# imedslab/OAProgressionMMF

Hardware: AMD Instinct MI355X
Metric: knees/sec full XR+MRI+clin fusion train step (higher is better)
Workload: dtype f32; 1 GPU; syn3: XR1MR3C1CnnTrf train step (fwd+FocalLoss+bwd+Adam), per-GPU batch 8, global batch 8, BASELINE config 4 on BASELINE's synthetic tensors: XR 1x310x310 + 3 x MRI 1x160x384x384 (slice-major) + 9 clinical; random-init weights; parallelism=dp1, activation_recompute=012,012,01

## Files before the change

### oaprogressionmmf_amd/csrc/koaf_conv.hip

```cpp
#include "koaf_common.h"

namespace {

inline int64_t rup32(int64_t v) { return (v + 31) / 32 * 32; }

inline void set_fimg(KoafGemm* g, const KoafWImg* w, int R, int64_t K) {
    g->fmt = 1;
    g->A.fscale = KOAF_ACT_SCALE;
    g->B.amax = w->amax;
    if (!w->f) return;
    g->B.kind = 2; g->B.gather = 0;
    g->B.planes = w->f; g->B.ld = rup32(K); g->B.plane_stride = (int64_t)R * g->B.ld;
}

inline void set_aplanes(KoafOperand* a, const uint16_t* planes, int64_t plane_elems) {
    a->kind = 2; a->planes = planes; a->plane_stride = plane_elems; a->zeros = planes + 2 * plane_elems;
    a->ptr = nullptr; a->ptr2 = nullptr; a->tf = 0; a->sc = a->sh = a->sc2 = nullptr;
}

inline void set_gather(KoafOperand* o, int gather, int H, int W, int C, int CS, int PH, int PW, int KH, int KW, int stride, int pad_h,
                       int pad_w) {
    o->gather = gather;
    o->H = H; o->W = W; o->C = C; o->CS = CS;
    o->PH = PH; o->PW = PW;
    o->KH = KH; o->KW = KW; o->stride = stride; o->pad = pad_h; o->pad_w = pad_w;
}

inline bool is_pointwise(int KH, int KW, int stride, int pad) { return KH == 1 && KW == 1 && stride == 1 && pad == 0; }

struct WgradPlan { int bm, bn, splitk; };
inline WgradPlan wgrad_plan(int M, int N, int64_t K, int ctap, int batch) {
    WgradPlan p;
    p.bn = (N >= 128 && (ctap % 4) == 0) ? 128 : 64;
    p.bm = (M >= 128) ? 128 : 64;
    int64_t tiles = cdiv64(M, p.bm) * cdiv64(N, p.bn) * batch;
    int64_t sk = 1024 / tiles;
    int64_t kmax = cdiv64(K, 512);
    if (sk > kmax) sk = kmax;
    if (sk < 1) sk = 1;
    if (sk > 4096) sk = 4096;
    if (sk > 8) {
        int64_t best = sk & ~7ll;
        double beff = 0.0;
        for (int64_t c = ((sk * 3 / 4) + 7) & ~7ll; c <= 2 * sk && c <= kmax && c <= 4096; c += 8) {
            const int64_t blocks = tiles * c;
            const double eff = (double)blocks / (double)(cdiv64(blocks, 512) * 512);
            if (eff > beff + 0.02) { beff = eff; best = c; }
        }
        sk = best;
    }
    p.splitk = (int)sk;
    return p;
}

__global__ void __launch_bounds__(256) slab_reduce_b_kernel(const float* __restrict__ slabs, int ns, int64_t n,
                                                            float* __restrict__ out) {
    const int64_t i = ((int64_t)blockIdx.x * 256 + threadIdx.x) * 4;
    if (i >= n) return;
    const float* sb = slabs + (int64_t)blockIdx.y * ns * n;
    v4f a = *(const v4f*)(sb + i);
    for (int s = 1; s < ns; ++s) a += *(const v4f*)(sb + (int64_t)s * n + i);
    *(v4f*)(out + (int64_t)blockIdx.y * n + i) = a;
}

__global__ void __launch_bounds__(256) gconv_expand_kernel(const float* __restrict__ w, float* __restrict__ wexp,
                                                           int C, int Cg, float* __restrict__ amax) {
    const int64_t total = (int64_t)C * 9 * 64;
    unsigned mb = 0u;
    for (int64_t i = (int64_t)blockIdx.x * 256 + threadIdx.x; i < total; i += (int64_t)gridDim.x * 256) {
        const int ci = (int)(i & 63);
        int64_t r = i >> 6;
        const int tap = (int)(r % 9);
        const int co = (int)(r / 9);
        const int col = co & 63;
        const int g0 = (col / Cg) * Cg;
        float v = 0.f;
        if (ci >= g0 && ci < g0 + Cg) v = w[((int64_t)co * 9 + tap) * Cg + (ci - g0)];
        wexp[i] = v;
        mb = max(mb, koaf_absbits(v));
    }
    if (amax != nullptr) block_amax_raise_bits(mb, amax);
}
__global__ void __launch_bounds__(256) gconv_compress_kernel(const float* __restrict__ dwexp, float* __restrict__ dw,
                                                             int C, int Cg) {
    const int64_t total = (int64_t)C * 9 * Cg;
    for (int64_t i = (int64_t)blockIdx.x * 256 + threadIdx.x; i < total; i += (int64_t)gridDim.x * 256) {
        const int cg = (int)(i % Cg);
        int64_t r = i / Cg;
        const int tap = (int)(r % 9);
        const int co = (int)(r / 9);
        const int g0 = ((co & 63) / Cg) * Cg;
        dw[i] = dwexp[((int64_t)co * 9 + tap) * 64 + g0 + cg];
    }
}

}

extern "C" int koaf_conv2d_fwd(const float* x, const float* w, float* y, int32_t N, int32_t H, int32_t W, int32_t Cin,
                               int32_t Cout, int32_t KH, int32_t KW, int32_t stride, int32_t pad, const float* in_sc,
                               const float* in_sh, float* stats, int32_t* stats_rows, const float* stats_shift,
                               const KoafWImg* wimg, const uint16_t* x_planes, const KoafTail* tail, const KoafEmit* emit,
                               int32_t act16, void* stream) {
    KOAF_REQUIRE((x || x_planes) && w && y && N > 0 && Cin % 32 == 0 && Cout % 4 == 0, "koaf_conv2d_fwd: bad args (Cin=%d Cout=%d)",
                 Cin, Cout);
    KOAF_REQUIRE(!tail || (tail->idt && x && in_sc && in_sh && !x_planes && is_pointwise(KH, KW, stride, pad) && wimg &&
                           wimg->amax && wimg->f && (tail->idt_sc == nullptr) == (tail->idt_sh == nullptr)),
                 "koaf_conv2d_fwd: the fused bottleneck tail serves 1x1 / stride-1 convolutions with weight plane images, from x / in_sc / in_sh");
    KOAF_REQUIRE((in_sc == nullptr) == (in_sh == nullptr), "koaf_conv2d_fwd: in_sc/in_sh come together");
    const int OH = conv_out(H, KH, stride, pad), OW = conv_out(W, KW, stride, pad);
    const int64_t M = (int64_t)N * OH * OW;
    KOAF_REQUIRE(M < (1ll << 31), "koaf_conv2d_fwd: too many output pixels");
    KoafGemm g;
    zero_gemm(&g);
    g.A.ptr = x;
    g.A.kind = 0;
    if (is_pointwise(KH, KW, stride, pad) && !x_planes) {
        g.A.gather = 0;
        g.A.ld = Cin;
    } else
        set_gather(&g.A, 1, H, W, Cin, Cin, OH, OW, KH, KW, stride, pad, pad);
    if (in_sc) { g.A.tf = 1; g.A.sc = in_sc; g.A.sh = in_sh; }
    if (tail) { g.A.tf = 3; g.A.ptr2 = tail->idt; g.A.side = tail->y_out; g.A.sc2 = tail->idt_sc; g.A.sh2 = tail->idt_sc ? tail->idt_sh : nullptr; }
    g.B.ptr = w;
    g.B.kind = 0;
    g.B.ld = (int64_t)KH * KW * Cin;
    g.M = (int)M; g.N = Cout; g.K = KH * KW * Cin;
    if (wimg && wimg->amax) set_fimg(&g, wimg, Cout, g.K);
    if (x_planes) {
        KOAF_REQUIRE(g.A.gather == 1 && g.B.kind == 2, "koaf_conv2d_fwd: x_planes serve the gathered kernels and need wimg->f");
        set_aplanes(&g.A, x_planes, (int64_t)N * H * W * Cin);
    }
    g.C = y; g.ldc = Cout;
    g.stats = stats;
    g.stats_shift = stats ? stats_shift : nullptr;
    g.act16 = act16 ? 1 : 0;
    if (emit) {
        KOAF_REQUIRE(emit->planes && emit->sc && emit->sh && (Cout % 8) == 0, "koaf_conv2d_fwd: emit needs planes / sc / sh and Cout %% 8 == 0");
        g.out_planes = emit->planes; g.out_sc = emit->sc; g.out_sh = emit->sh; g.out_ps = M * Cout;
    }
    if (stats_rows) *stats_rows = koaf_gemm_part_rows(&g);
    return koaf_gemm(&g, stream);
}

extern "C" int32_t koaf_conv2d_stats_rows(int64_t M, int32_t Cout) { return (int32_t)cdiv64(M, 64); }

static void set_apply(KoafOperand* a, const KoafBnApply* ap, int C) {
    a->ptr = ap->dz; a->ptr2 = ap->c; a->tf = 2;
    a->sc = ap->coef; a->sc2 = ap->coef + 2 * (int64_t)C; a->sh = ap->coef + 3 * (int64_t)C;
    a->amax = ap->amax;
}

static void set_bnb(KoafGemm* g, const KoafBnb* b, float* part) {
    if (!b) return;
    g->bnb_amax = b->dz_amax;
    g->bnb_mode = b->mode;
    g->bnb_c = b->c; g->bnb_y = b->y; g->bnb_sc = b->sc; g->bnb_sh = b->sh;
    g->bnb_mean = b->mean; g->bnb_invstd = b->invstd;
    g->bnb2_c = b->c2; g->bnb2_mean = b->mean2; g->bnb2_invstd = b->invstd2;
    g->bnb_part = part;
}

extern "C" int32_t koaf_conv2d_dgrad_bnb_rows(int32_t N, int32_t H, int32_t W, int32_t Cin, int32_t stride) {
    if (stride == 2) {
        int64_t r = 0;
        for (int py = 0; py < 2; ++py)
            for (int px = 0; px < 2; ++px) r += cdiv64((int64_t)N * ((H - py + 1) / 2) * ((W - px + 1) / 2), 64);
        return (int32_t)r;
    }
    return (int32_t)cdiv64((int64_t)N * H * W, 64);
}

extern "C" int koaf_conv2d_dgrad_bnb(const float* dy, const float* w, float* dx, int32_t N, int32_t H, int32_t W,
                                     int32_t Cin, int32_t Cout, int32_t KH, int32_t KW, int32_t stride, int32_t pad,
                                     const float* residual, const KoafBnb* bnb, float* part, int32_t* part_rows,
                                     const KoafWImg* wimg, const float* dy_amax, const KoafBnApply* dy_apply,
                                     const uint16_t* dy_planes, int32_t act16, void* stream) {
    KOAF_REQUIRE(!dy_planes || (wimg && wimg->amax && wimg->d && (dy_amax || dy_apply) && KH * KW > 1),
                 "koaf_conv2d_dgrad: dy_planes need the weight's D plane image, dy_amax and a gathered (KH*KW > 1) kernel");
    KOAF_REQUIRE((dy || dy_apply || dy_planes) && w && dx && N > 0 && Cout % 32 == 0 && Cin % 4 == 0, "koaf_conv2d_dgrad: bad args");
    KOAF_REQUIRE(!dy_apply || (dy_apply->dz && dy_apply->c && dy_apply->coef && dy_apply->amax && wimg && wimg->amax && wimg->d),
                 "koaf_conv2d_dgrad: dy_apply needs dz / c / coef / amax and the weight's D plane image");
    if (dy_apply) { dy = dy_apply->dz; dy_amax = dy_apply->amax; }
    if (bnb && bnb->dz_amax && hipMemsetAsync(bnb->dz_amax, 0, sizeof(float), (hipStream_t)stream) != hipSuccess) {
        koaf_set_error("koaf_conv2d_dgrad_bnb: memset failed");
        return KOAF_ELAUNCH;
    }
    const bool f16 = wimg && wimg->amax && dy_amax;
    const bool ps = f16 && wimg->d != nullptr;
    const uint16_t* w_dimg = ps ? wimg->d : nullptr;
    const int64_t dld = (int64_t)KH * KW * Cout, dps = (int64_t)Cin * dld;
    KOAF_REQUIRE(!bnb || (part && part_rows), "koaf_conv2d_dgrad_bnb: part / part_rows required");
    const int nsum = (bnb && bnb->c2) ? 3 : 2;
    int rows_done = 0;
    const int OH = conv_out(H, KH, stride, pad), OW = conv_out(W, KW, stride, pad);
    const int64_t M = (int64_t)N * H * W;
    KOAF_REQUIRE(M < (1ll << 31), "koaf_conv2d_dgrad: too many pixels");
    KoafGemm g;
    if (stride == 2) {
        for (int py = 0; py < 2; ++py)
            for (int px = 0; px < 2; ++px) {
                const int Hc = (H - py + 1) / 2, Wc = (W - px + 1) / 2;
                if (Hc <= 0 || Wc <= 0) continue;
                const int khs = (py + pad) & 1, kws = (px + pad) & 1;
                const int nkh = khs < KH ? (KH - khs + 1) / 2 : 0, nkw = kws < KW ? (KW - kws + 1) / 2 : 0;
                const int offy = (py + pad - khs) / 2, offx = (px + pad - kws) / 2;
                zero_gemm(&g);
                g.prec = 1;
                if (f16) { g.fmt = 1; g.A.amax = dy_amax; g.B.amax = wimg->amax; }
                g.A.ptr = dy; g.A.kind = 0;
                if (dy_apply) set_apply(&g.A, dy_apply, Cout);
                set_gather(&g.A, 2, OH, OW, Cout, Cout, Hc, Wc, nkh > 0 ? nkh : 1, nkw > 0 ? nkw : 1, 1, offy, offx);
                g.B.ptr = w + ((int64_t)khs * KW + kws) * Cin; g.B.kind = 1; g.B.gather = 3;
                g.B.C = Cout; g.B.ld = (int64_t)KH * KW * Cin;
                g.B.KW = g.A.KW; g.B.tap_stride = 2ll * Cin; g.B.tap_stride_h = 2ll * KW * Cin;
                if (ps) {
                    g.B.kind = 2; g.B.gather = 0;
                    g.B.planes = w_dimg + ((int64_t)khs * KW + kws) * Cout; g.B.ld = dld; g.B.plane_stride = dps;
                    g.B.tap_stride = 2ll * Cout; g.B.tap_stride_h = 2ll * KW * Cout;
                }
                if (dy_planes && nkh > 0 && nkw > 0) set_aplanes(&g.A, dy_planes, (int64_t)N * OH * OW * Cout);
                g.M = N * Hc * Wc; g.N = Cin; g.K = nkh * nkw * Cout;
                g.C = dx; g.ldc = Cin;
                g.residual = residual; g.ldr = Cin;
                g.cmap = 1; g.cm_PH = Hc; g.cm_PW = Wc; g.cm_H = H; g.cm_W = W; g.cm_py = py; g.cm_px = px;
                if (bnb) {
                    set_bnb(&g, bnb, part + (int64_t)rows_done * nsum * Cin);
                    rows_done += koaf_gemm_part_rows(&g);
                }
                g.act16 = act16 ? 2 : 0;
                int rc = koaf_gemm(&g, stream);
                if (rc != KOAF_OK) return rc;
            }
        if (part_rows) *part_rows = rows_done;
        return KOAF_OK;
    }
    zero_gemm(&g);
    g.prec = 1;
    if (f16) { g.fmt = 1; g.A.amax = dy_amax; g.B.amax = wimg->amax; }
    g.A.ptr = dy;
    g.A.kind = 0;
    if (dy_apply) set_apply(&g.A, dy_apply, Cout);
    g.B.ptr = w;
    g.B.kind = 1;
    if (is_pointwise(KH, KW, stride, pad)) {
        g.A.gather = 0;
        g.A.ld = Cout;
        g.B.gather = 0;
        g.B.ld = Cin;
    } else {
        set_gather(&g.A, 2, OH, OW, Cout, Cout, H, W, KH, KW, stride, pad, pad);
        g.B.gather = 3;
        g.B.C = Cout;
        g.B.ld = (int64_t)KH * KW * Cin;
        g.B.KW = KW;
        g.B.tap_stride = Cin;
        g.B.tap_stride_h = (int64_t)KW * Cin;
    }
    if (ps) {
        g.B.kind = 2; g.B.gather = 0; g.B.C = 0; g.B.tap_stride = g.B.tap_stride_h = 0;
        g.B.planes = w_dimg; g.B.ld = dld; g.B.plane_stride = dps;
    }
    if (dy_planes) set_aplanes(&g.A, dy_planes, (int64_t)N * OH * OW * Cout);
    g.M = (int)M; g.N = Cin; g.K = KH * KW * Cout;
    g.C = dx; g.ldc = Cin;
    g.residual = residual; g.ldr = Cin;
    if (bnb) {
        set_bnb(&g, bnb, part);
        *part_rows = koaf_gemm_part_rows(&g);
    }
    g.act16 = act16 ? 2 : 0;
    return koaf_gemm(&g, stream);
}

extern "C" int koaf_conv2d_dgrad(const float* dy, const float* w, float* dx, int32_t N, int32_t H, int32_t W,
                                 int32_t Cin, int32_t Cout, int32_t KH, int32_t KW, int32_t stride, int32_t pad,
                                 const float* residual, const KoafWImg* wimg, const float* dy_amax,
                                 const KoafBnApply* dy_apply, const uint16_t* dy_planes, int32_t act16, void* stream) {
    return koaf_conv2d_dgrad_bnb(dy, w, dx, N, H, W, Cin, Cout, KH, KW, stride, pad, residual, nullptr, nullptr,
                                 nullptr, wimg, dy_amax, dy_apply, dy_planes, act16, stream);
}

bool koaf_wgrad3_ring_ok(int N, int H, int W, int Cin, int Cout);
int64_t koaf_wgrad3_ring_ws(int N, int H, int W, int Cin, int Cout);
int koaf_wgrad3_ring(const uint16_t* dy_planes, const uint16_t* x_planes, float* dw, float* slabs, const float* dy_amax,
                     float x_scale, int N, int H, int W, int Cin, int Cout, void* stream);
static inline bool wgrad3_ring_shape(int N, int H, int W, int Cin, int Cout, int KH, int KW, int stride, int pad) {
    return KH == 3 && KW == 3 && stride == 1 && pad == 1 && koaf_wgrad3_ring_ok(N, H, W, Cin, Cout);
}

int koaf_wgrad1(const KoafGemm& g, int bm, int bn, void* stream);
constexpr int WGRAD1_MIN_KCHUNK = 1024;
static inline WgradPlan wgrad1_tile(const KoafGemm& g, const WgradPlan& p, bool pointwise) {
    WgradPlan t = {0, 0, p.splitk};
    if (!pointwise || g.fmt != 1 || g.act16 != 0 || g.A.kind != 1 || g.B.kind != 1) return t;
    if (g.M % 128 || g.N % 128 || (g.M < 256 && g.N < 256)) return t;
    const int bm = g.M >= 256 ? 256 : 128, bn = g.N >= 256 ? 256 : 128;
    if (g.M % bm || g.N % bn) return t;
    if (rup32(cdiv64(g.K, p.splitk)) < WGRAD1_MIN_KCHUNK) return t;
    if (!aligned16(g.A.ptr) || !aligned16(g.B.ptr) || !aligned16(g.C)) return t;
    if (g.A.tf && (!aligned16(g.A.ptr2) || !aligned16(g.A.sc) || !aligned16(g.A.sh) || !aligned16(g.A.sc2))) return t;
    if (g.B.tf && (!aligned16(g.B.sc) || !aligned16(g.B.sh))) return t;
    t.bm = bm; t.bn = bn;
    return t;
}

extern "C" int64_t koaf_conv2d_wgrad_ws(int32_t N, int32_t H, int32_t W, int32_t Cin, int32_t Cout, int32_t KH,
                                        int32_t KW, int32_t stride, int32_t pad) {
    const int OH = conv_out(H, KH, stride, pad), OW = conv_out(W, KW, stride, pad);
    WgradPlan p = wgrad_plan(Cout, KH * KW * Cin, (int64_t)N * OH * OW, Cin, 1);
    int64_t ws = p.splitk > 1 ? (int64_t)(p.splitk + 16) * Cout * KH * KW * Cin : 0;
    if (wgrad3_ring_shape(N, H, W, Cin, Cout, KH, KW, stride, pad)) {
        const int64_t w3 = koaf_wgrad3_ring_ws(N, H, W, Cin, Cout);
        if (w3 > ws) ws = w3;
    }
    return ws;
}

extern "C" int koaf_conv2d_wgrad(const float* dy, const float* x, float* dw, int32_t N, int32_t H, int32_t W,
                                 int32_t Cin, int32_t Cout, int32_t KH, int32_t KW, int32_t stride, int32_t pad,
                                 const float* in_sc, const float* in_sh, float* slabs, const float* dy_amax,
                                 const KoafBnApply* dy_apply, const uint16_t* dy_planes, const uint16_t* x_planes,
                                 int32_t act16, void* stream) {
    KOAF_REQUIRE((dy_planes == nullptr) == (x_planes == nullptr) && (!dy_planes || dy_amax || dy_apply),
                 "koaf_conv2d_wgrad: dy_planes and x_planes come together, with dy_amax (or dy_apply)");
    KOAF_REQUIRE((dy || dy_apply || dy_planes) && (x || x_planes) && dw && N > 0 && Cin % 64 == 0 && Cout % 4 == 0, "koaf_conv2d_wgrad: bad args");
    KOAF_REQUIRE(!dy_apply || (dy_apply->dz && dy_apply->c && dy_apply->coef && dy_apply->amax),
                 "koaf_conv2d_wgrad: dy_apply needs dz / c / coef / amax");
    if (dy_apply) { dy = dy_apply->dz; dy_amax = dy_apply->amax; }
    KOAF_REQUIRE((in_sc == nullptr) == (in_sh == nullptr), "koaf_conv2d_wgrad: in_sc/in_sh come together");
    const int OH = conv_out(H, KH, stride, pad), OW = conv_out(W, KW, stride, pad);
    const int64_t P = (int64_t)N * OH * OW;
    KOAF_REQUIRE(P < (1ll << 31), "koaf_conv2d_wgrad: too many pixels");
    const int Ntot = KH * KW * Cin;
    if (dy_planes && slabs && wgrad3_ring_shape(N, H, W, Cin, Cout, KH, KW, stride, pad))
        return koaf_wgrad3_ring(dy_planes, x_planes, dw, slabs, dy_amax, KOAF_ACT_SCALE, N, H, W, Cin, Cout, stream);
    WgradPlan p = wgrad_plan(Cout, Ntot, P, Cin, 1);
    KOAF_REQUIRE(p.splitk == 1 || slabs, "koaf_conv2d_wgrad: workspace required");
    KoafGemm g;
    zero_gemm(&g);
    g.prec = 1;
    if (dy_amax) { g.fmt = 1; g.A.amax = dy_amax; g.B.fscale = KOAF_ACT_SCALE; }
    g.A.ptr = dy; g.A.kind = 1; g.A.ld = Cout;
    if (dy_apply) set_apply(&g.A, dy_apply, Cout);
    g.B.ptr = x; g.B.kind = 1;
    if (is_pointwise(KH, KW, stride, pad)) {
        g.B.gather = 0;
        g.B.ld = Cin;
    } else
        set_gather(&g.B, 1, H, W, Cin, Cin, OH, OW, KH, KW, stride, pad, pad);
    if (in_sc) { g.B.tf = 1; g.B.sc = in_sc; g.B.sh = in_sh; }
    if (dy_planes) {
        set_aplanes(&g.A, dy_planes, P * Cout);
        g.A.kind = 3; g.A.ld = Cout;
        set_aplanes(&g.B, x_planes, (int64_t)N * H * W * Cin);
        g.B.kind = 3;
        set_gather(&g.B, 1, H, W, Cin, Cin, OH, OW, KH, KW, stride, pad, pad);
    }
    g.M = Cout; g.N = Ntot; g.K = (int)P;
    g.bm = p.bm; g.bn = p.bn; g.splitk = p.splitk;
    g.C = p.splitk > 1 ? slabs : dw;
    g.ldc = Ntot;
    g.act16 = (act16 && !dy_planes) ? 3 : 0;
    const WgradPlan t1 = wgrad1_tile(g, p, is_pointwise(KH, KW, stride, pad));
    int rc = t1.bm ? koaf_wgrad1(g, t1.bm, t1.bn, stream) : koaf_gemm(&g, stream);
    if (rc != KOAF_OK || p.splitk == 1) return rc;
    return koaf_slab_reduce(slabs, p.splitk, (int64_t)Cout * Ntot, dw, stream);
}

extern "C" int koaf_gconv_expand_w(const float* w, float* wexp, int32_t C, int32_t groups, float* amax, void* stream) {
    KOAF_REQUIRE(w && wexp && C % 64 == 0 && groups > 0 && C % groups == 0 && 64 % (C / groups) == 0,
                 "koaf_gconv_expand_w: C=%d groups=%d unsupported", C, groups);
    hipLaunchKernelGGL(gconv_expand_kernel, dim3(1024), dim3(256), 0, STREAM, w, wexp, C, C / groups, amax);
    return koaf_check_launch("koaf_gconv_expand_w");
}
extern "C" int koaf_gconv_compress_dw(const float* dwexp, float* dw, int32_t C, int32_t groups, void* stream) {
    KOAF_REQUIRE(dwexp && dw && C % 64 == 0 && groups > 0 && C % groups == 0 && 64 % (C / groups) == 0,
                 "koaf_gconv_compress_dw: C=%d groups=%d unsupported", C, groups);
    hipLaunchKernelGGL(gconv_compress_kernel, dim3(512), dim3(256), 0, STREAM, dwexp, dw, C, C / groups);
    return koaf_check_launch("koaf_gconv_compress_dw");
}

extern "C" int koaf_gconv3x3_fwd(const float* x, const float* wexp, float* y, int32_t N, int32_t H, int32_t W,
                                 int32_t C, int32_t stride, const float* in_sc, const float* in_sh, float* stats,
                                 int32_t* stats_rows, const float* stats_shift, const float* w_amax, int32_t act16, void* stream) {
    KOAF_REQUIRE(x && wexp && y && N > 0 && C % 64 == 0, "koaf_gconv3x3_fwd: bad args");
    const int OH = conv_out(H, 3, stride, 1), OW = conv_out(W, 3, stride, 1);
    const int64_t M = (int64_t)N * OH * OW;
    KOAF_REQUIRE(M < (1ll << 31), "koaf_gconv3x3_fwd: too many pixels");
    KoafGemm g;
    zero_gemm(&g);
    g.nb1 = C / 64;
    g.A.ptr = x; g.A.kind = 0; g.A.bs1 = 64;
    set_gather(&g.A, 1, H, W, 64, C, OH, OW, 3, 3, stride, 1, 1);
    if (in_sc) { g.A.tf = 1; g.A.sc = in_sc; g.A.sh = in_sh; }
    g.B.ptr = wexp; g.B.kind = 0; g.B.ld = 576; g.B.bs1 = 64 * 576;
    g.M = (int)M; g.N = 64; g.K = 576;
    g.C = y; g.ldc = C; g.cbs1 = 64;
    g.stats = stats; g.stats_ld = C; g.stats_bs = 64;
    g.stats_shift = stats ? stats_shift : nullptr;
    g.bn = 64; g.bm = 128;
    if (stats_rows) *stats_rows = (int)cdiv64(M, g.bm);
    g.A.tf_bs = 64;
    g.act16 = act16 ? 1 : 0;
    if (w_amax && !act16) { g.fmt = 1; g.A.fscale = KOAF_ACT_SCALE; g.B.amax = w_amax; }
    return koaf_gemm(&g, stream);
}

extern "C" int koaf_gconv3x3_dgrad(const float* dy, const float* wexp, float* dx, int32_t N, int32_t H, int32_t W,
                                   int32_t C, int32_t stride, const float* w_amax, const float* dy_amax, void* stream) {
    KOAF_REQUIRE(dy && wexp && dx && N > 0 && C % 64 == 0, "koaf_gconv3x3_dgrad: bad args");
    const int OH = conv_out(H, 3, stride, 1), OW = conv_out(W, 3, stride, 1);
    const int64_t M = (int64_t)N * H * W;
    KOAF_REQUIRE(M < (1ll << 31), "koaf_gconv3x3_dgrad: too many pixels");
    KoafGemm g;
    zero_gemm(&g);
    g.prec = 1;
    g.nb1 = C / 64;
    g.A.ptr = dy; g.A.kind = 0; g.A.bs1 = 64;
    set_gather(&g.A, 2, OH, OW, 64, C, H, W, 3, 3, stride, 1, 1);
    g.B.ptr = wexp; g.B.kind = 1; g.B.gather = 3; g.B.C = 64; g.B.ld = 576; g.B.tap_stride = 64;
    g.B.tap_stride_h = 3 * 64; g.B.KW = 3;
    g.B.bs1 = 64 * 576;
    g.M = (int)M; g.N = 64; g.K = 576;
    g.C = dx; g.ldc = C; g.cbs1 = 64;
    g.bn = 64; g.bm = 128;
    if (w_amax && dy_amax) { g.fmt = 1; g.A.amax = dy_amax; g.B.amax = w_amax; }
    return koaf_gemm(&g, stream);
}

extern "C" int64_t koaf_gconv3x3_wgrad_ws(int32_t N, int32_t H, int32_t W, int32_t C, int32_t stride) {
    const int OH = conv_out(H, 3, stride, 1), OW = conv_out(W, 3, stride, 1);
    WgradPlan p = wgrad_plan(64, 576, (int64_t)N * OH * OW, 64, C / 64);
    return (int64_t)p.splitk * C * 576;
}

extern "C" int koaf_gconv3x3_wgrad(const float* dy, const float* x, float* dwexp, int32_t N, int32_t H, int32_t W,
                                   int32_t C, int32_t stride, const float* in_sc, const float* in_sh, float* slabs,
                                   const float* dy_amax, int32_t act16, void* stream) {
    KOAF_REQUIRE(dy && x && dwexp && slabs && N > 0 && C % 64 == 0, "koaf_gconv3x3_wgrad: bad args");
    const int OH = conv_out(H, 3, stride, 1), OW = conv_out(W, 3, stride, 1);
    const int64_t P = (int64_t)N * OH * OW;
    KOAF_REQUIRE(P < (1ll << 31), "koaf_gconv3x3_wgrad: too many pixels");
    const int nz = C / 64;
    WgradPlan p = wgrad_plan(64, 576, P, 64, nz);
    {
        KoafGemm g;
        zero_gemm(&g);
        g.prec = 1;
        g.A.ptr = dy; g.A.kind = 1; g.A.ld = C; g.A.bs1 = 64;
        g.B.ptr = x; g.B.kind = 1; g.B.bs1 = 64;
        set_gather(&g.B, 1, H, W, 64, C, OH, OW, 3, 3, stride, 1, 1);
        if (in_sc) { g.B.tf = 1; g.B.sc = in_sc; g.B.sh = in_sh; g.B.tf_bs = 64; }
        g.M = 64; g.N = 576; g.K = (int)P;
        g.nb0 = 1; g.nb1 = nz;
        g.bm = 64; g.bn = 64; g.splitk = p.splitk;
        g.C = slabs;
        g.ldc = 576; g.cbs1 = 64 * 576;
        g.act16 = act16 ? 3 : 0;
        if (dy_amax && !act16) { g.fmt = 1; g.A.amax = dy_amax; g.B.fscale = KOAF_ACT_SCALE; }
        int rc = koaf_gemm(&g, stream);
        if (rc != KOAF_OK) return rc;
    }
    const int64_t n = 64 * 576;
    hipLaunchKernelGGL(slab_reduce_b_kernel, dim3((unsigned)cdiv64(n / 4, 256), nz), dim3(256), 0, STREAM, slabs,
                       p.splitk, n, dwexp);
    return koaf_check_launch("koaf_gconv3x3_wgrad");
}
```

### oaprogressionmmf_amd/csrc/koaf_wgrad1.hip

```cpp
#include <hip/hip_runtime.h>
#include <stdint.h>
#include <type_traits>
#include "koaf.h"
#include "koaf_pieces.h"

namespace {
struct Wg1Params {
    const float* a;
    const float* a2;
    const float* asc;
    const float* ash;
    const float* asc2;
    const float* a_amax;
    const float* b;
    const float* bsc;
    const float* bsh;
    float b_scale;
    float* out;
    uint32_t* status;
    int M, N, K, splitk;
};

constexpr int WG1_NT = 512;

template <int R, int TF>
struct Wg1Loader {
    static constexpr int NU = R / 64;
    static constexpr int CV = R / 4;
    static constexpr int RP = WG1_NT / CV;
    static constexpr int SK = R / 2 + 16;
    static constexpr int PL = plane_dwords(R, false);
    v4f r[NU];
    v4f r2[TF == 2 ? NU : 1];
    v4f ca, cb, ck;
    const float* src;
    const float* src2;
    float fsc;
    unsigned ld, col, kr;

    __device__ __forceinline__ void init(const float* p, const float* p2, const float* sc, const float* sh, const float* sc2,
                                         int c0, int ldim, float scale) {
        const unsigned t = threadIdx.x;
        src = p; src2 = p2;
        fsc = scale;
        ld = (unsigned)ldim;
        col = (unsigned)c0 + 4u * (t % CV);
        kr = t / CV;
        ca = cb = ck = (v4f){0.f, 0.f, 0.f, 0.f};
        if constexpr (TF != 0) {
            ca = *(const v4f*)(sc + col) * fsc;
            cb = *(const v4f*)(sh + col) * fsc;
            if constexpr (TF == 2) ck = *(const v4f*)(sc2 + col) * fsc;
        }
    }
    __device__ __forceinline__ void issue(int i, int k0, int K) {
        const int kb = min(k0, K - 1);
        const unsigned rowmax = (unsigned)(K - 1 - kb);
        const unsigned row = min(kr + (unsigned)(RP * i), rowmax);
        const unsigned off = __umul24(row, ld) + col;
        const int64_t base = (int64_t)kb * ld;
        r[i] = *(const v4f*)(src + base + off);
        if constexpr (TF == 2) r2[i] = *(const v4f*)(src2 + base + off);
    }
    template <bool FULL>
    __device__ __forceinline__ void convert(int i, int klim, unsigned* S) {
        constexpr float HMAX = 65504.f;
        const bool ok = FULL || (int)(kr + (unsigned)(RP * i)) < klim;
        v4f v;
#pragma unroll
        for (int j = 0; j < 4; ++j) {
            float x = r[i][j];
            if constexpr (TF == 1) {
                x = fmaf(x, ca[j], cb[j]);
                x = __builtin_amdgcn_fmed3f(x, 0.f, HMAX);
            } else if constexpr (TF == 2) {
                x = fmaf(ca[j], x, fmaf(-ck[j], r2[i][j], cb[j]));
                x = __builtin_amdgcn_fmed3f(x, -HMAX, HMAX);
            } else {
                x = __builtin_amdgcn_fmed3f(x * fsc, -HMAX, HMAX);
            }
            v[j] = ok ? x : 0.f;
        }
        unsigned pl[2][2];
        split2h(v, pl);
        const unsigned off = (kr + (unsigned)(RP * i)) * SK + 2u * (threadIdx.x % CV);
#pragma unroll
        for (int q = 0; q < 2; ++q) *(uint2*)&S[q * PL + off] = make_uint2(pl[q][0], pl[q][1]);
    }
};

template <int BM, int BN, int TFA, int TFB>
__global__ void __launch_bounds__(WG1_NT) wgrad1_kernel(const Wg1Params p) {
    constexpr int WGM = 4, WGN = 2;
    constexpr int WM = BM / WGM, WN = BN / WGN, TM = WM / 32, TN = WN / 32;
    typedef Wg1Loader<BM, TFA> LA;
    typedef Wg1Loader<BN, TFB> LB;
    constexpr int A_ELEMS = 2 * LA::PL, B_ELEMS = 2 * LB::PL, STAGE = A_ELEMS + B_ELEMS;
    static_assert(2 * STAGE * 4 <= 160 * 1024, "two stages of both operands in LDS");
    __shared__ __attribute__((aligned(16))) unsigned smem[2 * STAGE];

    const int ntn = p.N / BN;
    unsigned bid = blockIdx.x;
    int split = blockIdx.y;
    if (gridDim.y > 1 && (gridDim.y & 7) == 0) {
        const unsigned lin = blockIdx.x + gridDim.x * blockIdx.y, x = lin & 7, slot = lin >> 3;
        bid = slot % gridDim.x;
        split = (int)((slot / gridDim.x) * 8 + x);
    }
    const int tn = bid % ntn, tm = bid / ntn;
    const int m0 = tm * BM, n0 = tn * BN;
    const int kchunk = (((p.K + p.splitk - 1) / p.splitk + BK - 1) / BK) * BK;
    const int kbeg = split * kchunk;
    const int kend = min(p.K, kbeg + kchunk);
    const int klen = max(kend - kbeg, 0), nstep = (klen + BK - 1) / BK;

    const float sca = scale_of_amax(*p.a_amax), scb = p.b_scale;
    float alpha = 1.f / (sca * scb);
    if (!koaf_bits_finite(koaf_absbits(*p.a_amax))) {
        alpha = __uint_as_float(0x7fc00000u);
        if (blockIdx.x == 0 && blockIdx.y == 0 && threadIdx.x == 0) koaf_status_add(p.status, 1, 1u);
    }

    LA la;
    LB lb;
    la.init(p.a, p.a2, p.asc, p.ash, p.asc2, m0, p.M, sca);
    lb.init(p.b, nullptr, p.bsc, p.bsh, nullptr, n0, p.N, scb);

    const int t = threadIdx.x, lane = t & 63, w = t >> 6;
    const int wm = w / WGN, wn = w % WGN;

    v16f acc[TM][TN];
#pragma unroll
    for (int i = 0; i < TM; ++i)
#pragma unroll
        for (int j = 0; j < TN; ++j)
#pragma unroll
            for (int e = 0; e < 16; ++e) acc[i][j][e] = 0.f;

    constexpr int NUT = LA::NU + LB::NU, NG = 2 * TN;
    auto unit = [&](auto full, int u, int klim, unsigned* S, int k2) {
        constexpr bool FULL = decltype(full)::value;
        if (u < LA::NU) {
            la.template convert<FULL>(u, klim, S);
            la.issue(u, k2, p.K);
        } else {
            lb.template convert<FULL>(u - LA::NU, klim, S + A_ELEMS);
            lb.issue(u - LA::NU, k2, p.K);
        }
    };
    auto step = [&](auto full, int cur, int klim, int k2) {
        const unsigned* Au = smem + cur * STAGE;
        const unsigned* Bu = Au + A_ELEMS;
        unsigned* Sn = smem + (cur ^ 1) * STAGE;
#pragma unroll
        for (int g = 0; g < 2; ++g) {
            v4i ap[TM][2];
#pragma unroll
            for (int i = 0; i < TM; ++i)
#pragma unroll
                for (int q = 0; q < 2; ++q) ap[i][q] = frag_load<BM, false>(Au + q * LA::PL, wm * WM + 32 * i, g, lane);
#pragma unroll
            for (int jn = 0; jn < TN; ++jn) {
                v4i bp[2];
#pragma unroll
                for (int q = 0; q < 2; ++q) bp[q] = frag_load<BN, false>(Bu + q * LB::PL, wn * WN + 32 * jn, g, lane);
                constexpr int PAH[3] = {1, 0, 0}, PBH[3] = {0, 1, 0};
#pragma unroll
                for (int term = 0; term < 3; ++term)
#pragma unroll
                    for (int i = 0; i < TM; ++i)
                        acc[i][jn] = __builtin_amdgcn_mfma_f32_32x32x16_f16(__builtin_bit_cast(h16x8, ap[i][PAH[term]]),
                                                                            __builtin_bit_cast(h16x8, bp[PBH[term]]), acc[i][jn], 0, 0, 0);
                const int grp = g * TN + jn;
#pragma unroll
                for (int u = 0; u < NUT; ++u)
                    if (u * NG / NUT == grp) unit(full, u, klim, Sn, k2);
                __builtin_amdgcn_sched_barrier(0x104);
            }
        }
        asm volatile("s_waitcnt lgkmcnt(0)\n\ts_barrier" ::: "memory");
    };

    if (nstep > 0) {
#pragma unroll
        for (int i = 0; i < LA::NU; ++i) la.issue(i, kbeg, p.K);
#pragma unroll
        for (int i = 0; i < LB::NU; ++i) lb.issue(i, kbeg, p.K);
#pragma unroll
        for (int u = 0; u < NUT; ++u) unit(std::false_type{}, u, klen, smem, kbeg + BK);
        asm volatile("s_waitcnt lgkmcnt(0)\n\ts_barrier" ::: "memory");
    }
    const int nfull = max(klen / BK - 1, 0);
    int s = 0;
#pragma unroll 1
    for (; s < nfull; ++s) step(std::true_type{}, s & 1, BK, kbeg + (s + 2) * BK);
#pragma unroll 1
    for (; s < nstep; ++s) step(std::false_type{}, s & 1, klen - (s + 1) * BK, kbeg + (s + 2) * BK);

    float* out = p.out + (p.splitk > 1 ? (int64_t)split * p.M * p.N : (int64_t)0);
    const int r = lane & 31, h = lane >> 5;
#pragma unroll
    for (int i = 0; i < TM; ++i)
#pragma unroll
        for (int jn = 0; jn < TN; ++jn)
#pragma unroll
            for (int e = 0; e < 16; ++e) {
                float v = alpha * acc[i][jn][e];
                asm volatile("" : "+v"(v));
                v += 0.f;
                const int row = m0 + wm * WM + 32 * i + (e & 3) + 8 * (e >> 2) + 4 * h;
                const int col = n0 + wn * WN + 32 * jn + r;
                out[(int64_t)row * p.N + col] = v;
            }
}

template <int BM, int BN>
int wg1_launch(const Wg1Params& p, int tfa, int tfb, dim3 grid, hipStream_t s) {
#define WG1_GO(TA, TB) hipLaunchKernelGGL((wgrad1_kernel<BM, BN, TA, TB>), grid, dim3(WG1_NT), 0, s, p)
    if (tfa == 2) { if (tfb) WG1_GO(2, 1); else WG1_GO(2, 0); }
    else { if (tfb) WG1_GO(0, 1); else WG1_GO(0, 0); }
#undef WG1_GO
    return koaf_check_launch("koaf_wgrad1");
}
}

void koaf_log_launch(const char* variant, const KoafGemm& g, dim3 grid, dim3 launched);

int koaf_wgrad1(const KoafGemm& g, int bm, int bn, void* stream) {
    KOAF_REQUIRE(g.fmt == 1 && g.act16 == 0 && g.A.kind == 1 && g.B.kind == 1 && !g.A.gather && !g.B.gather && g.A.amax && g.A.ptr && g.B.ptr &&
                 g.C && (g.A.tf == 0 || (g.A.tf == 2 && g.A.ptr2 && g.A.sc && g.A.sh && g.A.sc2)) && (g.B.tf == 0 || (g.B.tf == 1 && g.B.sc && g.B.sh)) &&
                 (bm == 256 || bm == 128) && (bn == 256 || bn == 128) && bm + bn >= 384 && g.M % bm == 0 && g.N % bn == 0 && g.K >= BK && g.K < (1 << 30) &&
                 g.splitk >= 1 && g.splitk <= 65535 && g.A.ld == g.M && g.B.ld == g.N && g.ldc == g.N,
                 "koaf_wgrad1: bad args");
    Wg1Params p;
    p.a = g.A.ptr; p.a2 = g.A.ptr2; p.asc = g.A.sc; p.ash = g.A.sh; p.asc2 = g.A.sc2; p.a_amax = g.A.amax;
    p.b = g.B.ptr; p.bsc = g.B.sc; p.bsh = g.B.sh;
    p.b_scale = g.B.fscale != 0.f ? g.B.fscale : 1.f;
    p.out = g.C;
    p.status = g.status ? g.status : koaf_status_ptr();
    p.M = g.M; p.N = g.N; p.K = g.K; p.splitk = g.splitk;
    const dim3 grid((unsigned)((g.M / bm) * (g.N / bn)), (unsigned)g.splitk);
    KoafGemm rec = g;
    rec.bm = bm; rec.bn = bn;
    koaf_log_launch("koaf_wgrad1", rec, grid, grid);
    hipStream_t s = (hipStream_t)stream;
    if (bm == 256 && bn == 256) return wg1_launch<256, 256>(p, g.A.tf, g.B.tf, grid, s);
    if (bm == 256) return wg1_launch<256, 128>(p, g.A.tf, g.B.tf, grid, s);
    return wg1_launch<128, 256>(p, g.A.tf, g.B.tf, grid, s);
}
```

Measured before the change: 4.125 knees/s.

## Extend wgrad1 kernel to stride-2 implicit-gather convolutions via LDS row table

Lets the specialized wgrad1 weight-gradient kernel handle stride-2 1x1 and 3x3 convolutions with implicit im2col gather, not just pointwise ones. Each block precomputes a small ring of source-row offsets in LDS, rotating through four BK-sized slots, and marks padding rows invalid so the loader zero-fills them. These layers previously fell back to the generic gemm path. The cost is extra LDS, per-step index computation and a new template variant.

Result: faster. 4.179 knees/s (median of 6 runs) (+1.3%).

```diff
diff --git a/oaprogressionmmf_amd/csrc/koaf_conv.hip b/oaprogressionmmf_amd/csrc/koaf_conv.hip
--- a/oaprogressionmmf_amd/csrc/koaf_conv.hip
+++ b/oaprogressionmmf_amd/csrc/koaf_conv.hip
@@ -290,12 +290,18 @@
 
 int koaf_wgrad1(const KoafGemm& g, int bm, int bn, void* stream);
 constexpr int WGRAD1_MIN_KCHUNK = 1024;
-static inline WgradPlan wgrad1_tile(const KoafGemm& g, const WgradPlan& p, bool pointwise) {
+static inline WgradPlan wgrad1_tile(const KoafGemm& g, const WgradPlan& p) {
     WgradPlan t = {0, 0, p.splitk};
-    if (!pointwise || g.fmt != 1 || g.act16 != 0 || g.A.kind != 1 || g.B.kind != 1) return t;
+    const KoafOperand& B = g.B;
+    if (g.fmt != 1 || g.act16 != 0 || g.A.kind != 1 || B.kind != 1 || g.A.gather || (B.gather != 0 && B.gather != 1)) return t;
     if (g.M % 128 || g.N % 128 || (g.M < 256 && g.N < 256)) return t;
     const int bm = g.M >= 256 ? 256 : 128, bn = g.N >= 256 ? 256 : 128;
     if (g.M % bm || g.N % bn) return t;
+    if (B.gather == 1) {
+        const bool f11 = B.KH == 1 && B.KW == 1 && B.pad == 0 && B.pad_w == 0, f33 = B.KH == 3 && B.KW == 3 && B.pad == 1 && B.pad_w == 1;
+        if (B.stride != 2 || !(f11 || f33) || B.CS != B.C || B.C % bn || B.PH <= 0 || B.PW <= 0) return t;
+        if ((int64_t)(g.K / (B.PH * B.PW)) * B.H * B.W >= (1ll << 31)) return t;
+    }
     if (rup32(cdiv64(g.K, p.splitk)) < WGRAD1_MIN_KCHUNK) return t;
     if (!aligned16(g.A.ptr) || !aligned16(g.B.ptr) || !aligned16(g.C)) return t;
     if (g.A.tf && (!aligned16(g.A.ptr2) || !aligned16(g.A.sc) || !aligned16(g.A.sh) || !aligned16(g.A.sc2))) return t;
@@ -361,7 +367,7 @@
     g.C = p.splitk > 1 ? slabs : dw;
     g.ldc = Ntot;
     g.act16 = (act16 && !dy_planes) ? 3 : 0;
-    const WgradPlan t1 = wgrad1_tile(g, p, is_pointwise(KH, KW, stride, pad));
+    const WgradPlan t1 = wgrad1_tile(g, p);
     int rc = t1.bm ? koaf_wgrad1(g, t1.bm, t1.bn, stream) : koaf_gemm(&g, stream);
     if (rc != KOAF_OK || p.splitk == 1) return rc;
     return koaf_slab_reduce(slabs, p.splitk, (int64_t)Cout * Ntot, dw, stream);
diff --git a/oaprogressionmmf_amd/csrc/koaf_wgrad1.hip b/oaprogressionmmf_amd/csrc/koaf_wgrad1.hip
--- a/oaprogressionmmf_amd/csrc/koaf_wgrad1.hip
+++ b/oaprogressionmmf_amd/csrc/koaf_wgrad1.hip
@@ -19,11 +19,15 @@
     float* out;
     uint32_t* status;
     int M, N, K, splitk;
+    int H, W, C, PH, PW, KW, stride, pad, pad_w;
 };
 
 constexpr int WG1_NT = 512;
 
-template <int R, int TF>
+constexpr int WG1_TAB = 4 * BK;
+constexpr unsigned WG1_INVALID = 0x80000000u;
+
+template <int R, int TF, bool G = false>
 struct Wg1Loader {
     static constexpr int NU = R / 64;
     static constexpr int CV = R / 4;
@@ -37,6 +41,7 @@
     const float* src2;
     float fsc;
     unsigned ld, col, kr;
+    unsigned vm;
 
     __device__ __forceinline__ void init(const float* p, const float* p2, const float* sc, const float* sh, const float* sc2,
                                          int c0, int ldim, float scale) {
@@ -46,6 +51,7 @@
         ld = (unsigned)ldim;
         col = (unsigned)c0 + 4u * (t % CV);
         kr = t / CV;
+        vm = 0u;
         ca = cb = ck = (v4f){0.f, 0.f, 0.f, 0.f};
         if constexpr (TF != 0) {
             ca = *(const v4f*)(sc + col) * fsc;
@@ -62,10 +68,16 @@
         r[i] = *(const v4f*)(src + base + off);
         if constexpr (TF == 2) r2[i] = *(const v4f*)(src2 + base + off);
     }
+    __device__ __forceinline__ void issue_g(int i, const unsigned* T) {
+        const unsigned e = T[kr + (unsigned)(RP * i)];
+        vm = (vm & ~(1u << i)) | ((e >> 31) << i);
+        const uint64_t off = (uint64_t)(e & ~WG1_INVALID) * ld + col;
+        r[i] = *(const v4f*)(src + off);
+    }
     template <bool FULL>
     __device__ __forceinline__ void convert(int i, int klim, unsigned* S) {
         constexpr float HMAX = 65504.f;
-        const bool ok = FULL || (int)(kr + (unsigned)(RP * i)) < klim;
+        const bool ok = G ? ((vm >> i) & 1u) == 0u : (FULL || (int)(kr + (unsigned)(RP * i)) < klim);
         v4f v;
 #pragma unroll
         for (int j = 0; j < 4; ++j) {
@@ -89,15 +101,16 @@
     }
 };
 
-template <int BM, int BN, int TFA, int TFB>
+template <int BM, int BN, int TFA, int TFB, bool GB>
 __global__ void __launch_bounds__(WG1_NT) wgrad1_kernel(const Wg1Params p) {
     constexpr int WGM = 4, WGN = 2;
     constexpr int WM = BM / WGM, WN = BN / WGN, TM = WM / 32, TN = WN / 32;
     typedef Wg1Loader<BM, TFA> LA;
-    typedef Wg1Loader<BN, TFB> LB;
+    typedef Wg1Loader<BN, TFB, GB> LB;
     constexpr int A_ELEMS = 2 * LA::PL, B_ELEMS = 2 * LB::PL, STAGE = A_ELEMS + B_ELEMS;
-    static_assert(2 * STAGE * 4 <= 160 * 1024, "two stages of both operands in LDS");
-    __shared__ __attribute__((aligned(16))) unsigned smem[2 * STAGE];
+    static_assert((2 * STAGE + WG1_TAB) * 4 <= 160 * 1024, "two stages of both operands in LDS");
+    __shared__ __attribute__((aligned(16))) unsigned smem[2 * STAGE + (GB ? WG1_TAB : 0)];
+    [[maybe_unused]] unsigned* const tab = smem + 2 * STAGE;
 
     const int ntn = p.N / BN;
     unsigned bid = blockIdx.x;
@@ -124,7 +137,22 @@
     LA la;
     LB lb;
     la.init(p.a, p.a2, p.asc, p.ash, p.asc2, m0, p.M, sca);
-    lb.init(p.b, nullptr, p.bsc, p.bsh, nullptr, n0, p.N, scb);
+    [[maybe_unused]] int g_kh = 0, g_kw = 0;
+    if constexpr (GB) {
+        const int tap = n0 / p.C;
+        g_kh = tap / p.KW;
+        g_kw = tap - g_kh * p.KW;
+        lb.init(p.b, nullptr, p.bsc, p.bsh, nullptr, n0 - tap * p.C, p.C, scb);
+    } else
+        lb.init(p.b, nullptr, p.bsc, p.bsh, nullptr, n0, p.N, scb);
+    [[maybe_unused]] auto table = [&](int j, int lane32) {
+        const int k = kbeg + j * BK + lane32;
+        const unsigned kk = (unsigned)min(k, p.K - 1), ppi = (unsigned)(p.PH * p.PW);
+        const unsigned n = kk / ppi, rem = kk - n * ppi, oy = rem / (unsigned)p.PW, ox = rem - oy * (unsigned)p.PW;
+        const int sy = (int)oy * p.stride - p.pad + g_kh, sx = (int)ox * p.stride - p.pad_w + g_kw;
+        const bool ok = k < kend && (unsigned)sy < (unsigned)p.H && (unsigned)sx < (unsigned)p.W;
+        tab[(j & 3) * BK + lane32] = ok ? (n * (unsigned)p.H + (unsigned)sy) * (unsigned)p.W + (unsigned)sx : WG1_INVALID;
+    };
 
     const int t = threadIdx.x, lane = t & 63, w = t >> 6;
     const int wm = w / WGN, wn = w % WGN;
@@ -145,13 +173,17 @@
             la.issue(u, k2, p.K);
         } else {
             lb.template convert<FULL>(u - LA::NU, klim, S + A_ELEMS);
-            lb.issue(u - LA::NU, k2, p.K);
+            if constexpr (GB) lb.issue_g(u - LA::NU, tab + (((k2 - kbeg) / BK) & 3) * BK);
+            else lb.issue(u - LA::NU, k2, p.K);
         }
     };
     auto step = [&](auto full, int cur, int klim, int k2) {
         const unsigned* Au = smem + cur * STAGE;
         const unsigned* Bu = Au + A_ELEMS;
         unsigned* Sn = smem + (cur ^ 1) * STAGE;
+        if constexpr (GB) {
+            if (threadIdx.x < BK) table((k2 - kbeg) / BK + 1, threadIdx.x);
+        }
 #pragma unroll
         for (int g = 0; g < 2; ++g) {
             v4i ap[TM][2];
@@ -182,10 +214,17 @@
     };
 
     if (nstep > 0) {
+        if constexpr (GB) {
+            if (threadIdx.x < 3 * BK) table(threadIdx.x / BK, threadIdx.x % BK);
+            asm volatile("s_waitcnt lgkmcnt(0)\n\ts_barrier" ::: "memory");
+        }
 #pragma unroll
         for (int i = 0; i < LA::NU; ++i) la.issue(i, kbeg, p.K);
 #pragma unroll
-        for (int i = 0; i < LB::NU; ++i) lb.issue(i, kbeg, p.K);
+        for (int i = 0; i < LB::NU; ++i) {
+            if constexpr (GB) lb.issue_g(i, tab);
+            else lb.issue(i, kbeg, p.K);
+        }
 #pragma unroll
         for (int u = 0; u < NUT; ++u) unit(std::false_type{}, u, klen, smem, kbeg + BK);
         asm volatile("s_waitcnt lgkmcnt(0)\n\ts_barrier" ::: "memory");
@@ -214,37 +253,49 @@
             }
 }
 
-template <int BM, int BN>
+template <int BM, int BN, bool GB>
 int wg1_launch(const Wg1Params& p, int tfa, int tfb, dim3 grid, hipStream_t s) {
-#define WG1_GO(TA, TB) hipLaunchKernelGGL((wgrad1_kernel<BM, BN, TA, TB>), grid, dim3(WG1_NT), 0, s, p)
+#define WG1_GO(TA, TB) hipLaunchKernelGGL((wgrad1_kernel<BM, BN, TA, TB, GB>), grid, dim3(WG1_NT), 0, s, p)
     if (tfa == 2) { if (tfb) WG1_GO(2, 1); else WG1_GO(2, 0); }
     else { if (tfb) WG1_GO(0, 1); else WG1_GO(0, 0); }
 #undef WG1_GO
     return koaf_check_launch("koaf_wgrad1");
 }
+template <bool GB>
+int wg1_tile(const Wg1Params& p, int bm, int bn, int tfa, int tfb, dim3 grid, hipStream_t s) {
+    if (bm == 256 && bn == 256) return wg1_launch<256, 256, GB>(p, tfa, tfb, grid, s);
+    if (bm == 256) return wg1_launch<256, 128, GB>(p, tfa, tfb, grid, s);
+    return wg1_launch<128, 256, GB>(p, tfa, tfb, grid, s);
+}
 }
 
 void koaf_log_launch(const char* variant, const KoafGemm& g, dim3 grid, dim3 launched);
 
 int koaf_wgrad1(const KoafGemm& g, int bm, int bn, void* stream) {
-    KOAF_REQUIRE(g.fmt == 1 && g.act16 == 0 && g.A.kind == 1 && g.B.kind == 1 && !g.A.gather && !g.B.gather && g.A.amax && g.A.ptr && g.B.ptr &&
-                 g.C && (g.A.tf == 0 || (g.A.tf == 2 && g.A.ptr2 && g.A.sc && g.A.sh && g.A.sc2)) && (g.B.tf == 0 || (g.B.tf == 1 && g.B.sc && g.B.sh)) &&
+    const KoafOperand& B = g.B;
+    const bool gb = B.gather == 1;
+    KOAF_REQUIRE(g.fmt == 1 && g.act16 == 0 && g.A.kind == 1 && B.kind == 1 && !g.A.gather && (B.gather == 0 || gb) && g.A.amax && g.A.ptr && B.ptr &&
+                 g.C && (g.A.tf == 0 || (g.A.tf == 2 && g.A.ptr2 && g.A.sc && g.A.sh && g.A.sc2)) && (B.tf == 0 || (B.tf == 1 && B.sc && B.sh)) &&
                  (bm == 256 || bm == 128) && (bn == 256 || bn == 128) && bm + bn >= 384 && g.M % bm == 0 && g.N % bn == 0 && g.K >= BK && g.K < (1 << 30) &&
-                 g.splitk >= 1 && g.splitk <= 65535 && g.A.ld == g.M && g.B.ld == g.N && g.ldc == g.N,
+                 g.splitk >= 1 && g.splitk <= 65535 && g.A.ld == g.M && (gb || B.ld == g.N) && g.ldc == g.N,
                  "koaf_wgrad1: bad args");
+    KOAF_REQUIRE(!gb || (B.stride == 2 && B.KH == B.KW && B.pad == B.pad_w && ((B.KH == 1 && B.pad == 0) || (B.KH == 3 && B.pad == 1)) &&
+                         (B.CS == 0 || B.CS == B.C) && B.C % bn == 0 && g.N == B.KH * B.KW * B.C && B.PH > 0 && B.PW > 0 &&
+                         B.PH == (B.H + 2 * B.pad - B.KH) / 2 + 1 && B.PW == (B.W + 2 * B.pad_w - B.KW) / 2 + 1 && g.K % (B.PH * B.PW) == 0 &&
+                         (int64_t)(g.K / (B.PH * B.PW)) * B.H * B.W < (1ll << 31)),
+                 "koaf_wgrad1: bad gather");
     Wg1Params p;
     p.a = g.A.ptr; p.a2 = g.A.ptr2; p.asc = g.A.sc; p.ash = g.A.sh; p.asc2 = g.A.sc2; p.a_amax = g.A.amax;
-    p.b = g.B.ptr; p.bsc = g.B.sc; p.bsh = g.B.sh;
-    p.b_scale = g.B.fscale != 0.f ? g.B.fscale : 1.f;
+    p.b = B.ptr; p.bsc = B.sc; p.bsh = B.sh;
+    p.b_scale = B.fscale != 0.f ? B.fscale : 1.f;
     p.out = g.C;
     p.status = g.status ? g.status : koaf_status_ptr();
     p.M = g.M; p.N = g.N; p.K = g.K; p.splitk = g.splitk;
+    p.H = B.H; p.W = B.W; p.C = B.C; p.PH = B.PH; p.PW = B.PW; p.KW = B.KW; p.stride = B.stride; p.pad = B.pad; p.pad_w = B.pad_w;
     const dim3 grid((unsigned)((g.M / bm) * (g.N / bn)), (unsigned)g.splitk);
     KoafGemm rec = g;
     rec.bm = bm; rec.bn = bn;
     koaf_log_launch("koaf_wgrad1", rec, grid, grid);
     hipStream_t s = (hipStream_t)stream;
-    if (bm == 256 && bn == 256) return wg1_launch<256, 256>(p, g.A.tf, g.B.tf, grid, s);
-    if (bm == 256) return wg1_launch<256, 128>(p, g.A.tf, g.B.tf, grid, s);
-    return wg1_launch<128, 256>(p, g.A.tf, g.B.tf, grid, s);
-}
+    return gb ? wg1_tile<true>(p, bm, bn, g.A.tf, B.tf, grid, s) : wg1_tile<false>(p, bm, bn, g.A.tf, B.tf, grid, s);
+}
```
